# AliaksandrSiarohin/wc-gan

Hardware: AMD Instinct MI355X
Metric: images/sec G+D step, CIFAR-10 ResNet-SN+WC, batch 64 (higher is better)
Workload: dtype f32; 1 GPU; CIFAR-10 ResNet SN uncond + WC (scripts/cifar10_resnet_sn_uncond.sh), batch 64/GPU, training_ratio 5, generator_batch_multiple 2; parallelism=dp1, wc_statistics=per-replica, launch=hipgraph

## Files before the change

### include/wc_hip.h

```cpp
#ifndef WC_HIP_H
#define WC_HIP_H

#include <stddef.h>
#include <stdint.h>

#ifdef __cplusplus
extern "C" {
#endif

#define WC_ABI_VERSION 8

#define WC_OK                 0
#define WC_ERR_NULL          -1
#define WC_ERR_SHAPE         -2
#define WC_ERR_CHANNELS      -3
#define WC_ERR_WORKSPACE     -4
#define WC_ERR_ARG           -5

typedef void* wc_stream_t;

int         wc_abi_version(void);
const char* wc_error_string(int code);

#define WC_CORE_API "wc_stats_f32 wc_factor_f64 wc_color_f32 wc_group_bias_f32 wc_apply_f32 wc_apply_act_f32 " \
// ... 234 lines not shown

#define WC_CONV_SCRATCH_BYTES 2048

int wc_conv_supported(const wc_conv_geom* g);

int wc_conv_split_f32(const float* x, int64_t n, int relu, void* hi, void* lo, float* scale, void* amax_scratch,
                      wc_stream_t stream);

#define WC_CONV_COLSUM_ROWS 512
int wc_conv_split_colsum_f32(const float* x, int64_t n, int relu, void* hi, void* lo, float* scale, void* amax_scratch,
                             float* colsum_partials, int C, wc_stream_t stream);

#define WC_CONV_HIST_FLOATS (4 * 512 + 16)
#define WC_CONV_HIST_REDO (4 * 512)
int wc_conv_split_hist_f32(const float* x, int64_t n, int relu, void* hi, void* lo, float* scale, float* colsum_partials , int C,
                           float* hist, int bootstrap, wc_stream_t stream);

size_t wc_conv_weights_bytes(const wc_conv_geom* g);
int wc_conv_weights_f32(const float* w, int64_t stride_k, int64_t stride_n, int64_t stride_r, int64_t stride_s,
                        int64_t n_elems, const wc_conv_geom* g, void* image, float* scale, void* amax_scratch,
                        const float* known_amax, int known_count, wc_stream_t stream);

int wc_conv_weights_pair_f32(const float* w, int64_t stride_r, int64_t stride_s, int64_t n_elems,
                             int64_t a_stride_k, int64_t a_stride_n, const wc_conv_geom* ga, void* image_a,
                             int64_t b_stride_k, int64_t b_stride_n, const wc_conv_geom* gb, void* image_b,
                             float* scale, void* amax_scratch, const float* known_amax, int known_count,
                             wc_stream_t stream);

size_t wc_conv_workspace_bytes(const wc_conv_geom* g);
int wc_conv_f16x3(const void* xhi, const void* xlo, const float* xscale, const void* wimage, const float* wscale,
                  const float* bias, const void* zero_line, const wc_conv_geom* g, int relu, float* y,
                  void* ws, size_t ws_bytes, wc_stream_t stream);

size_t wc_conv_wrw_workspace_bytes(const wc_conv_geom* g);
int wc_conv_wrw_f16x3(const void* xhi, const void* xlo, const float* xscale, const void* ghi, const void* glo,
                      const float* gscale, const void* zero_line, const wc_conv_geom* g, float* dw, int64_t stride_k,
                      int64_t stride_n, int64_t stride_r, int64_t stride_s, void* ws, size_t ws_bytes,
                      wc_stream_t stream);

int    wc_conv_wrw_narrow_supported(int64_t N, int64_t H, int64_t W, int Cin, int Cout, int ksize);
size_t wc_conv_wrw_narrow_workspace_bytes(int64_t N, int64_t H, int64_t W, int Cin, int Cout, int ksize);
int    wc_conv_wrw_narrow_f32(const float* x, const float* gy, int64_t N, int64_t H, int64_t W, int Cin, int Cout, int ksize,
                              float* dw, int64_t stride_k, int64_t stride_n, int64_t stride_r, int64_t stride_s, float* db ,
                              void* ws, size_t ws_bytes, wc_stream_t stream);

int    wc_conv_fwd_narrow_f32(const float* x, const float* w, int64_t stride_k, int64_t stride_n, int64_t stride_r, int64_t stride_s,
                              const float* bias , int64_t N, int64_t H, int64_t W, int Cin, int Cout, int ksize, int relu,
                              float* y, wc_stream_t stream);

int wc_conv_wrw_bias_f16x3(const void* xhi, const void* xlo, const float* xscale, const void* ghi, const void* glo,
                           const float* gscale, const void* zero_line, const wc_conv_geom* g, float* dw, int64_t stride_k,
                           int64_t stride_n, int64_t stride_r, int64_t stride_s, const float* colsum_partials, float* db,
                           void* ws, size_t ws_bytes, wc_stream_t stream);

int wc_stream_copy_f32(const float* src, float* dst, int64_t n, wc_stream_t stream);

#ifdef __cplusplus
}
#endif
#endif
```

### wc_gan_amd/_lib.py

```python
from __future__ import annotations

import ctypes
import os
from ctypes import c_float, c_char_p, c_double, c_int, c_int64, c_size_t, c_void_p

_HERE = os.path.dirname(os.path.abspath(__file__))
LIB_PATH = os.path.join(_HERE, "libwc_hip.so")

WC_OK = 0
ABI_VERSION = 8
ERRORS = {-1: "WC_ERR_NULL", -2: "WC_ERR_SHAPE", -3: "WC_ERR_CHANNELS", -4: "WC_ERR_WORKSPACE", -5: "WC_ERR_ARG"}

SIGNATURES = {
    "wc_abi_version": (c_int, []),
    "wc_error_string": (c_char_p, [c_int]),
    "wc_stats_workspace_bytes": (c_size_t, [c_int64, c_int, c_int]),
    "wc_factor_workspace_bytes": (c_size_t, [c_int, c_int]),
    "wc_color_workspace_bytes": (c_size_t, [c_int, c_int]),
    "wc_bwd_reduce_workspace_bytes": (c_size_t, [c_int64, c_int64, c_int, c_int, c_int]),
    "wc_bwd_factor_workspace_bytes": (c_size_t, [c_int, c_int]),
    "wc_apply_workspace_bytes": (c_size_t, [c_int64, c_int64, c_int, c_int]),
    "wc_apply_plan_bytes": (c_size_t, [c_int, c_int]),
    "wc_bwd_apply_workspace_bytes": (c_size_t, [c_int64, c_int64, c_int, c_int]),
    "wc_stats_f32": (c_int, [c_void_p, c_int64, c_int, c_int, c_void_p, c_void_p, c_void_p, c_size_t, c_void_p]),
# ... 90 lines not shown
    "wc_stream_copy_f32": (c_int, [c_void_p, c_void_p, c_int64, c_void_p]),
    "wc_spectral_norm_workspace_bytes": (c_size_t, [c_int, c_int]),
    "wc_spectral_norm_batched_f32": (c_int, [c_void_p, c_int, c_int, c_float, c_void_p]),
    "wc_spectral_norm_bwd_batched_f32": (c_int, [c_void_p, c_int, c_int, c_void_p]),
    "wc_spectral_norm_f32": (c_int, [c_void_p, c_int, c_int, c_void_p, c_void_p, c_int, c_float, c_void_p, c_void_p,
                                     c_void_p, c_void_p, c_void_p, c_size_t, c_void_p]),
    "wc_spectral_norm_bwd_f32": (c_int, [c_void_p, c_void_p, c_void_p, c_void_p, c_void_p, c_int, c_int, c_int, c_void_p,
                                         c_void_p, c_size_t, c_void_p]),
    "wc_conv_supported": (c_int, [c_void_p]),
    "wc_conv_split_f32": (c_int, [c_void_p, c_int64, c_int, c_void_p, c_void_p, c_void_p, c_void_p, c_void_p]),
    "wc_conv_weights_bytes": (c_size_t, [c_void_p]),
    "wc_conv_weights_f32": (c_int, [c_void_p, c_int64, c_int64, c_int64, c_int64, c_int64, c_void_p, c_void_p, c_void_p,
                                    c_void_p, c_void_p, c_int, c_void_p]),
    "wc_spectral_norm_amax_offset": (c_size_t, [c_int, c_int]),
    "wc_spectral_norm_error_offset": (c_size_t, [c_int, c_int]),
    "wc_conv_split_hist_f32": (c_int, [c_void_p, c_int64, c_int, c_void_p, c_void_p, c_void_p, c_void_p, c_int, c_void_p, c_int, c_void_p]),
    "wc_conv_fwd_narrow_f32": (c_int, [c_void_p, c_void_p, c_int64, c_int64, c_int64, c_int64, c_void_p, c_int64, c_int64, c_int64, c_int, c_int, c_int,
                                       c_int, c_void_p, c_void_p]),
    "wc_conv_wrw_narrow_supported": (c_int, [c_int64, c_int64, c_int64, c_int, c_int, c_int]),
    "wc_conv_wrw_narrow_workspace_bytes": (c_size_t, [c_int64, c_int64, c_int64, c_int, c_int, c_int]),
    "wc_conv_wrw_narrow_f32": (c_int, [c_void_p, c_void_p, c_int64, c_int64, c_int64, c_int, c_int, c_int, c_void_p, c_int64, c_int64, c_int64,
                                       c_int64, c_void_p, c_void_p, c_size_t, c_void_p]),
    "wc_conv_split_colsum_f32": (c_int, [c_void_p, c_int64, c_int, c_void_p, c_void_p, c_void_p, c_void_p, c_void_p, c_int, c_void_p]),
    "wc_conv_wrw_bias_f16x3": (c_int, [c_void_p, c_void_p, c_void_p, c_void_p, c_void_p, c_void_p, c_void_p, c_void_p, c_void_p,
                                       c_int64, c_int64, c_int64, c_int64, c_void_p, c_void_p, c_void_p, c_size_t, c_void_p]),
    "wc_conv_weights_pair_f32": (c_int, [c_void_p, c_int64, c_int64, c_int64, c_int64, c_int64, c_void_p, c_void_p,
                                         c_int64, c_int64, c_void_p, c_void_p, c_void_p, c_void_p, c_void_p, c_int, c_void_p]),
    "wc_conv_wrw_workspace_bytes": (c_size_t, [c_void_p]),
    "wc_conv_wrw_f16x3": (c_int, [c_void_p, c_void_p, c_void_p, c_void_p, c_void_p, c_void_p, c_void_p, c_void_p, c_void_p,
                                  c_int64, c_int64, c_int64, c_int64, c_void_p, c_size_t, c_void_p]),
    "wc_conv_workspace_bytes": (c_size_t, [c_void_p]),
    "wc_conv_f16x3": (c_int, [c_void_p, c_void_p, c_void_p, c_void_p, c_void_p, c_void_p, c_void_p, c_void_p, c_int,
                              c_void_p, c_void_p, c_size_t, c_void_p]),
}



class SnItem(ctypes.Structure):
    _fields_ = [("W", c_void_p), ("u", c_void_p), ("v", c_void_p), ("w_sn", c_void_p), ("sigma", c_void_p),
                ("u_used", c_void_p), ("v_used", c_void_p), ("ws", c_void_p), ("rows", c_int), ("cols", c_int)]


class SnBwdItem(ctypes.Structure):
    _fields_ = [("g", c_void_p), ("w_sn", c_void_p), ("u", c_void_p), ("v", c_void_p), ("sigma", c_void_p),
                ("dW", c_void_p), ("ws", c_void_p), ("rows", c_int), ("cols", c_int)]


class ConvGeom(ctypes.Structure):
    _fields_ = [("N", c_int), ("H", c_int), ("W", c_int), ("Hin", c_int), ("Win", c_int), ("Cin", c_int),
                ("Hout", c_int), ("Wout", c_int), ("Cout", c_int), ("in_stride", c_int), ("out_stride", c_int),
                ("ntaps", c_int), ("nphase", c_int),
                ("dy", (ctypes.c_byte * 16) * 4), ("dx", (ctypes.c_byte * 16) * 4),
                ("off_y", ctypes.c_byte * 4), ("off_x", ctypes.c_byte * 4),
                ("nsrc", (ctypes.c_byte * 16) * 4),
                ("wr", ((ctypes.c_byte * 4) * 16) * 4), ("ws", ((ctypes.c_byte * 4) * 16) * 4),
                ("wcoef", c_float)]


_lib = None


class WcHipError(RuntimeError):
    pass


def shared_gpu_guard(device_count=None) -> bool:
# ... 53 lines not shown
```

### wc_gan_amd/conv.py

```python
from __future__ import annotations

import ctypes
import os

import torch
import torch.nn.functional as F

from . import _lib, _state
from .ops import _ptr, _stream

_zero_lines = {}


def _zero_line(device):
    z = _zero_lines.get(device)
    if z is None:
        z = _zero_lines[device] = torch.zeros(64, dtype=torch.uint8, device=device)
    return z


def _plain(r, s):
    return [(r, s)], 1.0


# ... 32 lines not shown


def _phase_geom(N, Hin, Win, Cin, Cout, source=_plain):
    g = _lib.ConvGeom()
    g.N, g.Hin, g.Win, g.Cin, g.Cout = N, Hin, Win, Cin, Cout
    g.H, g.W, g.Hout, g.Wout = Hin, Win, 2 * Hin, 2 * Win
    g.in_stride, g.out_stride, g.ntaps, g.nphase = 1, 2, 4, 4
    for py in range(2):
        for px in range(2):
            p = py * 2 + px
            g.off_y[p], g.off_x[p] = py, px
            t = 0
            for dy in ((-1, 0) if py == 0 else (0, 1)):
                for dx in ((-1, 0) if px == 0 else (0, 1)):
                    g.dy[p][t], g.dx[p][t] = dy, dx
                    _set_sources(g, p, t, py + 1 - 2 * dy, px + 1 - 2 * dx, source)
                    t += 1
    return g


def _supported(g):
    return bool(_lib.load().wc_conv_supported(ctypes.addressof(g)))


def supported(x, w, kind):
    handed = getattr(x, '_wc_planes', None) is not None
    if not (x.is_cuda and x.dtype == torch.float32 and x.dim() == 4 and (handed or x.is_contiguous()) and w.dtype == torch.float32):
        return False
    p = _plan(kind, x, w)
    return bool(p) and p.ok


class _Plan:
    __slots__ = ('ok', 'fwd', 'bwd', 'fwd_ws', 'bwd_ws', 'wrw_ws', 'fwd_ptr', 'bwd_ptr')

    def __init__(self, kind, N, H, W, wshape):
        class _W:
            shape = wshape
        lib = _lib.load()
        (gf, kf, nf), (gb, kb, nb) = _geoms(kind, N, H, W, _W)
        self.fwd, self.bwd = (gf, kf, nf), (gb, kb, nb)
        self.fwd_ptr, self.bwd_ptr = ctypes.addressof(gf), ctypes.addressof(gb)
        self.ok = bool(lib.wc_conv_supported(self.fwd_ptr)) and bool(lib.wc_conv_supported(self.bwd_ptr))
        self.fwd_ws = lib.wc_conv_workspace_bytes(self.fwd_ptr) if self.ok else 0
        self.bwd_ws = lib.wc_conv_workspace_bytes(self.bwd_ptr) if self.ok else 0
        self.wrw_ws = lib.wc_conv_wrw_workspace_bytes(self.fwd_ptr) if self.ok else 0


_plans = {}


def _plan(kind, x, w):
    key = (kind, tuple(x.shape), tuple(w.shape))
    p = _plans.get(key)
    if p is None:
        N, H, W, C = x.shape
        good = (kind == 'same' and w.shape[1] == C and w.shape[2] == w.shape[3] and w.shape[2] in (1, 3)) or \
               (kind == 'down' and w.shape[1] == C and tuple(w.shape[2:]) == (4, 4) and H % 2 == 0 and W % 2 == 0) or \
               (kind == 'down3' and w.shape[1] == C and tuple(w.shape[2:]) == (3, 3) and H % 2 == 0 and W % 2 == 0) or \
               (kind == 'up3' and w.shape[1] == C and tuple(w.shape[2:]) == (3, 3)) or \
               (kind == 'up' and w.shape[0] == C and tuple(w.shape[2:]) == (4, 4))
        if kind not in ('same', 'down', 'up', 'down3', 'up3'):
            raise ValueError(kind)
        p = _plans[key] = _Plan(kind, N, H, W, tuple(w.shape)) if good else False
    return p


def _colsum_ok(C):
    return C % 4 == 0 and 256 % (C // 4) == 0


SPLIT_HIST = os.environ.get('WC_SPLIT_HIST', '1') != '0'
HIST_FLOATS = 4 * 512 + 16
HIST_REDO = 4 * 512


_REDO_MODE = os.environ.get('WC_SPLIT_HIST_REDO', '1')


# ... 51 lines not shown
    ext = _storage_extent(w)
    if ext != w.numel():
        raise ValueError("weight must be dense")
    known = getattr(w, '_wc_amax', None)
    _lib.check(lib.wc_conv_weights_f32(_ptr(w), w.stride(k_axis), w.stride(n_axis), w.stride(2), w.stride(3), ext,
                                       ctypes.addressof(geom), _ptr(img), _ptr(scale), scale.data_ptr() + 4,
                                       _ptr(known), 0 if known is None else known.numel(), _stream()),
               "wc_conv_weights_f32")
    return img, scale


def weight_image_pair(w, fwd, bwd):
    lib = _lib.load()
    (ga, ka, na), (gb, kb, nb) = fwd, bwd
    img_a = torch.empty(lib.wc_conv_weights_bytes(ctypes.addressof(ga)), dtype=torch.uint8, device=w.device)
    img_b = torch.empty(lib.wc_conv_weights_bytes(ctypes.addressof(gb)), dtype=torch.uint8, device=w.device)
    scale = torch.empty(2 + 512, dtype=torch.float32, device=w.device)
    ext = _storage_extent(w)
    if ext != w.numel():
        raise ValueError("weight must be dense")
    known = getattr(w, '_wc_amax', None)
    _lib.check(lib.wc_conv_weights_pair_f32(_ptr(w), w.stride(2), w.stride(3), ext,
                                            w.stride(ka), w.stride(na), ctypes.addressof(ga), _ptr(img_a),
                                            w.stride(kb), w.stride(nb), ctypes.addressof(gb), _ptr(img_b),
                                            _ptr(scale), scale.data_ptr() + 8, _ptr(known), 0 if known is None else known.numel(),
                                            _stream()), "wc_conv_weights_pair_f32")
    return (img_a, scale[0:1]), (img_b, scale[1:2])


def _cached_image(w, key, geom, k_axis, n_axis):
    return weight_image(w, geom, k_axis, n_axis)


def run(planes, image, geom, bias=None, relu=False, nbytes=None):
    hi, lo, xs = planes
    img, ws = image
    lib = _lib.load()
    y = torch.empty((geom.N, geom.Hout, geom.Wout, geom.Cout), dtype=torch.float32, device=hi.device)
    if nbytes is None:
        nbytes = lib.wc_conv_workspace_bytes(ctypes.addressof(geom))
    work = torch.empty(nbytes, dtype=torch.uint8, device=hi.device) if nbytes else None
    _lib.check(lib.wc_conv_f16x3(_ptr(hi), _ptr(lo), _ptr(xs), _ptr(img), _ptr(ws), _ptr(bias) if bias is not None else None,
                                 _ptr(_zero_line(hi.device)), ctypes.addressof(geom), 1 if relu else 0, _ptr(y),
                                 _ptr(work), nbytes, _stream()), "wc_conv_f16x3")
    return y


def _geoms(kind, N, H, W, w):
    if kind == 'same':
        co, ci, k = w.shape[0], w.shape[1], w.shape[2]
        fwd = _dense_geom(N, H, W, ci, co, k, 1)
        bwd = _dense_geom(N, H, W, co, ci, k, 1)
        for t in range(k * k):
            bwd.dy[0][t], bwd.dx[0][t] = -bwd.dy[0][t], -bwd.dx[0][t]
        return (fwd, 1, 0), (bwd, 0, 1)
    if kind in ('down', 'down3'):
        co, ci = w.shape[0], w.shape[1]
        src = _pooled3 if kind == 'down3' else _plain
        return (_dense_geom(N, H, W, ci, co, 4, 2, src), 1, 0), (_phase_geom(N, H // 2, W // 2, co, ci, src), 0, 1)
    if kind == 'up3':
        co, ci = w.shape[0], w.shape[1]
        return (_phase_geom(N, H, W, ci, co, _upsampled3), 1, 0), (_dense_geom(N, 2 * H, 2 * W, co, ci, 4, 2, _upsampled3), 0, 1)
    ci, co = w.shape[0], w.shape[1]
    return (_phase_geom(N, H, W, ci, co), 0, 1), (_dense_geom(N, 2 * H, 2 * W, co, ci, 4, 2), 1, 0)


def weight_gradient(x_planes, g_planes, geom, w, k_axis, n_axis, nbytes=None, colsum=None):
    lib = _lib.load()
    xh, xl, xs = x_planes
    gh, gl, gs = g_planes[:3]
    dw = torch.empty_like(w)
    if dw.stride() != w.stride():
        raise ValueError("weight must be dense")
    if nbytes is None:
        nbytes = lib.wc_conv_wrw_workspace_bytes(ctypes.addressof(geom))
    ws = torch.empty(nbytes, dtype=torch.uint8, device=w.device)
    if colsum is not None:
        db = torch.empty(geom.Cout, dtype=torch.float32, device=w.device)
        _lib.check(lib.wc_conv_wrw_bias_f16x3(_ptr(xh), _ptr(xl), _ptr(xs), _ptr(gh), _ptr(gl), _ptr(gs), _ptr(_zero_line(w.device)),
                                              ctypes.addressof(geom), _ptr(dw), w.stride(k_axis), w.stride(n_axis), w.stride(2),
                                              w.stride(3), _ptr(colsum), _ptr(db), _ptr(ws), nbytes, _stream()),
                   "wc_conv_wrw_bias_f16x3")
        return dw, db
    _lib.check(lib.wc_conv_wrw_f16x3(_ptr(xh), _ptr(xl), _ptr(xs), _ptr(gh), _ptr(gl), _ptr(gs), _ptr(_zero_line(w.device)),
                                     ctypes.addressof(geom), _ptr(dw), w.stride(k_axis), w.stride(n_axis), w.stride(2),
                                     w.stride(3), _ptr(ws), nbytes, _stream()), "wc_conv_wrw_f16x3")
    return dw


def takes_planes(shape, wshape, kind):
    class _S:
        pass
    xs, ws = _S(), _S()
    xs.shape, ws.shape = tuple(shape), tuple(wshape)
    p = _plan(kind, xs, ws)
    return bool(p) and p.ok


class _FastConv(torch.autograd.Function):
    @staticmethod
    def forward(ctx, x, w, bias, kind, plan, relu_input=False, handed=None, site=None):
        gf, kf, nf = plan.fwd
        planes = handed if handed is not None else split_planes(x, relu=relu_input, site=site, role='x')
        ctx.site = site
        if ctx.needs_input_grad[0]:
            img, ctx.bwd_image = weight_image_pair(w, plan.fwd, plan.bwd)
        else:
            img, ctx.bwd_image = weight_image(w, gf, kf, nf), None
        y = run(planes, img, gf, bias, nbytes=plan.fwd_ws)
        ctx.save_for_backward(w, *planes, *((x,) if relu_input else ()))
        ctx.kind, ctx.has_bias, ctx.plan, ctx.relu_input = kind, bias is not None, plan, relu_input
        return y

    @staticmethod
    def backward(ctx, gy):
        w, xh, xl, xs = ctx.saved_tensors[:4]
        kind, plan = ctx.kind, ctx.plan
        gy = gy.contiguous()
        want_db = ctx.has_bias and ctx.needs_input_grad[2]
        fused_db = want_db and ctx.needs_input_grad[1] and _colsum_ok(gy.shape[-1])
        g_planes = split_planes(gy, colsum=fused_db, site=ctx.site, role='g')
        dx = dw = db = None
        if ctx.needs_input_grad[0]:
            gb, kb, nb = plan.bwd
            image = ctx.bwd_image if ctx.bwd_image is not None else weight_image(w, gb, kb, nb)
            dx = run(g_planes[:3], image, gb, nbytes=plan.bwd_ws)
            if ctx.relu_input:
                dx = torch.ops.aten.threshold_backward(dx, ctx.saved_tensors[4], 0)
        if ctx.needs_input_grad[1]:
            gf, kf, nf = plan.fwd
            if fused_db:
                dw, db = weight_gradient((xh, xl, xs), g_planes, gf, w, kf, nf, nbytes=plan.wrw_ws, colsum=g_planes[3])
            else:
                dw = weight_gradient((xh, xl, xs), g_planes, gf, w, kf, nf, nbytes=plan.wrw_ws)
        if want_db and not fused_db:
            db = gy.sum((0, 1, 2))
        return dx, dw, db, None, None, None, None, None


_ones = {}


def _one(device):
    t = _ones.get(device)
    if t is None:
        t = torch.ones(1, dtype=torch.float32, device=device)
        if not torch.cuda.is_current_stream_capturing():
            _ones[device] = t
    return t


class _SplitConv(torch.autograd.Function):

    @staticmethod
    def forward(ctx, x, w, bias, plan, st, site=None):
        from . import ops
        ctx.site = site
        gf, kf, nf = plan.fwd
        wf, bf = ops.fold_channel_scale(w, bias, st.scale, st.center)
        img = weight_image(wf, gf, kf, nf)
        ctx.bwd_image = None
        if ctx.needs_input_grad[0]:
            gb, kb, nb = plan.bwd
            ctx.bwd_image = weight_image(w, gb, kb, nb)
        hi, lo = st.planes[0].view(st.shape), st.planes[1].view(st.shape)
        one = _one(hi.device)
        y = run((hi, lo, one), img, gf, bf, nbytes=plan.fwd_ws)
        ctx.save_for_backward(w, hi, lo, one, st.scale, st.center)
        ctx.plan, ctx.has_bias = plan, bias is not None
        return y

    @staticmethod
    def backward(ctx, gy):
        from . import ops
        w, xh, xl, one, scale, center = ctx.saved_tensors
        plan = ctx.plan
        gy = gy.contiguous()
        need_w = ctx.needs_input_grad[1]
        need_b = ctx.has_bias and ctx.needs_input_grad[2]
        fused_db = need_w and _colsum_ok(gy.shape[-1])
        g_planes = split_planes(gy, colsum=fused_db, site=ctx.site, role='g')
        dx = dw = db = None
        if ctx.needs_input_grad[0]:
            gb, kb, nb = plan.bwd
            image = ctx.bwd_image if ctx.bwd_image is not None else weight_image(w, gb, kb, nb)
            dx = run(g_planes[:3], image, gb, nbytes=plan.bwd_ws)
        if need_w:
            gf, kf, nf = plan.fwd
            if fused_db:
                D, db = weight_gradient((xh, xl, one), g_planes, gf, w, kf, nf, nbytes=plan.wrw_ws, colsum=g_planes[3])
            else:
                D = weight_gradient((xh, xl, one), g_planes, gf, w, kf, nf, nbytes=plan.wrw_ws)
                db = gy.sum((0, 1, 2))
            dw = ops.unfold_channel_scale(D, db, scale, center)
        elif need_b:
            db = gy.sum((0, 1, 2))
        return dx, dw, (db if need_b else None), None, None, None


def split_conv(x, st, w, bias=None, site=None):
    p = _plan('same', x, w)
    if not (p and p.ok and tuple(w.shape[2:]) == (1, 1) and w.dtype == torch.float32):
        raise _lib.WcHipError(f"split_conv: a pre-split handle reached a convolution without a planes path {tuple(x.shape)} x {tuple(w.shape)}")
    return _SplitConv.apply(x, w, bias, p, st, site)


def fast_conv_or_none(x, w, bias=None, kind='same', relu_input=False, site=None):
    handed = getattr(x, '_wc_planes', None)
    if not supported(x, w, kind):
        if handed is not None:
            raise _lib.WcHipError(f"fast_conv: a K3 handle reached a convolution that cannot take planes {tuple(x.shape)} x {tuple(w.shape)} ({kind})")
        return None
    if handed is not None:
        if relu_input:
            raise ValueError("a K3 handle is already ReLU'd")
        return _FastConv.apply(x, w, bias, kind, _plan(kind, x, w), False, handed, site)
    return _FastConv.apply(x, w, bias, kind, _plan(kind, x, w), relu_input, None, site)


# ... 100 lines not shown
```

### wc_gan_amd/csrc/wc_conv.hip

```cpp
#include "wc_common.h"
#include "../../include/wc_hip.h"
#include <stdlib.h>


namespace {

constexpr int kMaxTaps = 16, kMaxPhase = 4;

struct ConvArgs {
    const _Float16* xhi; const _Float16* xlo;
    const _Float16* zero;
    const char* wimg;
    const float* xscale; const float* wscale;
    const float* bias;
    float* y;
    int N, H, W, Hin, Win, Cin, Cout, in_stride, ntaps, nphase, Hout, Wout, out_stride, relu;
    unsigned magHW, shHW, magW, shW;
    int ksplit; float* partial;
    signed char dy[kMaxPhase][kMaxTaps], dx[kMaxPhase][kMaxTaps];
    signed char offy[kMaxPhase], offx[kMaxPhase];
};

__device__ __forceinline__ void lds_dma16(const void* g, unsigned lds)
{
    unsigned keep;
    asm volatile("s_mov_b32 %0, m0\n\ts_mov_b32 m0, %2\n\ts_nop 0\n\tglobal_load_lds_dwordx4 %1, off\n\ts_mov_b32 m0, %0"
                 : "=&s"(keep) : "v"(g), "s"(lds) : "memory");
}

template <int MB, int NB, bool KS>
__global__ __launch_bounds__(256) void conv_f16x3_kernel(ConvArgs a)
{
    extern __shared__ __attribute__((aligned(16))) char smem[];
    constexpr int TM = 64 * MB, TN = 64 * NB;
    constexpr int A_BYTES = 2 * MB * 4 * 1024, B_BYTES = 2 * NB * 4 * 1024, STAGE = A_BYTES + B_BYTES;
    constexpr int AQ = (2 * MB) / 4;
    static_assert(AQ >= 1, "MB >= 2");

    const int tid = threadIdx.x, lane = tid & 63;
    const int wave = __builtin_amdgcn_readfirstlane(tid >> 6);
    const int wm = wave >> 1, wn = wave & 1;
    const int ntn = a.Cout / TN;
    const int phase = blockIdx.y / ntn, nt = blockIdx.y - phase * ntn;
    const unsigned m0 = blockIdx.x * TM;
    const unsigned HW = a.H * a.W;
    const int koff = (lane >> 5) * 8;

    int gy[AQ], gx[AQ];
    unsigned gpix[AQ];
    #pragma unroll
    for (int q = 0; q < AQ; ++q) {
        const unsigned m = m0 + (wave * AQ + q) * 32 + (lane & 31);
        const unsigned n = __umulhi(m, a.magHW) >> a.shHW, rem = m - n * HW;
        const unsigned yy = __umulhi(rem, a.magW) >> a.shW, xx = rem - yy * a.W;
        gy[q] = yy * a.in_stride; gx[q] = xx * a.in_stride; gpix[q] = n * (a.Hin * a.Win);
    }
    const unsigned lds0 = (unsigned)(size_t)((__attribute__((address_space(3))) char*)smem);
    const int nchunk = a.Cin >> 5;
    const int iters = a.ntaps * nchunk;
    const int nblk_all = a.Cout >> 5;
// ... 98 lines not shown
            #pragma unroll
            for (int g = 0; g < PER; ++g) {
                const int prod = g / (MB * NB), i = (g / NB) % MB, j = g % NB;
                acc[i][j] = __builtin_amdgcn_mfma_f32_32x32x16_f16(fa[ks][i][prod == 0 ? 1 : 0], fb[ks][j][prod == 1 ? 1 : 0], acc[i][j], 0, 0, 0);
                if ((g + 1) % GAP == 0) {
                    dma(ks * HALF + g / GAP);
                    __builtin_amdgcn_sched_barrier(0);
                }
                if (ks == 0 && g == PER / 2) {
                    frags(stage, 1);
                    __builtin_amdgcn_sched_barrier(0);
                }
            }
        }
    }
    __builtin_amdgcn_s_waitcnt(0x0F70);
    const float inv = 1.0f / (a.xscale[0] * a.wscale[0]);
    const int oy0 = a.offy[phase], ox0 = a.offx[phase];
    float bj[NB];
    #pragma unroll
    for (int j = 0; j < NB; ++j) bj[j] = a.bias ? a.bias[nt * TN + (wn * NB + j) * 32 + (lane & 31)] : 0.f;
    #pragma unroll
    for (int i = 0; i < MB; ++i) {
        #pragma unroll
        for (int r = 0; r < 16; ++r) {
            const unsigned row = (r & 3) + 8 * (r >> 2) + 4 * (lane >> 5);
            const unsigned m = m0 + (wm * MB + i) * 32 + row;
            const unsigned n = __umulhi(m, a.magHW) >> a.shHW, rem = m - n * HW;
            const unsigned yy = __umulhi(rem, a.magW) >> a.shW, xx = rem - yy * a.W;
            const int64_t opix = ((int64_t)n * a.Hout + (yy * a.out_stride + oy0)) * a.Wout + (xx * a.out_stride + ox0);
            const int64_t oe = opix * a.Cout + nt * TN + wn * NB * 32 + (lane & 31);
            if (KS) {
                float* o = a.partial + (int64_t)blockIdx.z * ((int64_t)a.N * a.Hout * a.Wout * a.Cout) + oe;
                #pragma unroll
                for (int j = 0; j < NB; ++j) o[j * 32] = acc[i][j][r];
            } else {
                float* o = a.y + oe;
                #pragma unroll
                for (int j = 0; j < NB; ++j) {
                    float v = acc[i][j][r] * inv + bj[j];
                    if (a.relu) v = fmaxf(v, 0.f);
                    o[j * 32] = v;
                }
            }
        }
    }
}

__global__ __launch_bounds__(256) void conv_ksplit_reduce_kernel(const float* __restrict__ partial, int ksplit, int64_t n4, int cout,
                                                                 const float* __restrict__ xscale, const float* __restrict__ wscale,
                                                                 const float* __restrict__ bias, int relu, float* __restrict__ y)
{
    const float inv = 1.0f / (xscale[0] * wscale[0]);
    for (int64_t i = (int64_t)blockIdx.x * 256 + threadIdx.x; i < n4; i += (int64_t)gridDim.x * 256) {
        f32x4 v = *reinterpret_cast<const f32x4*>(partial + 4 * i);
        int z = 1;
        for (; z + 3 < ksplit; z += 4) {
            f32x4 t[4];
            #pragma unroll
            for (int u = 0; u < 4; ++u) t[u] = *reinterpret_cast<const f32x4*>(partial + 4 * ((z + u) * n4 + i));
            #pragma unroll
            for (int u = 0; u < 4; ++u) v += t[u];
        }
        for (; z < ksplit; ++z) v += *reinterpret_cast<const f32x4*>(partial + 4 * (z * n4 + i));
        v = v * inv;
        if (bias) v += *reinterpret_cast<const f32x4*>(bias + (4 * i) % cout);
        if (relu) { v[0] = fmaxf(v[0], 0.f); v[1] = fmaxf(v[1], 0.f); v[2] = fmaxf(v[2], 0.f); v[3] = fmaxf(v[3], 0.f); }
        *reinterpret_cast<f32x4*>(y + 4 * i) = v;
    }
}

constexpr int kAmaxBlocks = 512;

__global__ __launch_bounds__(256) void conv_absmax_kernel(const float* __restrict__ x, int64_t n4, int64_t n, float* __restrict__ partial,
                                                          float* __restrict__ colsum = nullptr, int c4n = 0)
{
    __shared__ float red[4];
    __shared__ f32x4 red4[256];
    float m = 0.f;
    f32x4 cs = {0.f, 0.f, 0.f, 0.f};
    for (int64_t i = blockIdx.x * 256 + threadIdx.x; i < n4; i += (int64_t)gridDim.x * 256) {
        const f32x4 v = *reinterpret_cast<const f32x4*>(x + 4 * i);
        m = fmaxf(fmaxf(m, fabsf(v[0])), fmaxf(fabsf(v[1]), fmaxf(fabsf(v[2]), fabsf(v[3]))));
        cs += v;
    }
    if (blockIdx.x == 0 && threadIdx.x == 0) for (int64_t i = 4 * n4; i < n; ++i) m = fmaxf(m, fabsf(x[i]));
    #pragma unroll
    for (int o = 32; o > 0; o >>= 1) m = fmaxf(m, __shfl_xor(m, o));
    if ((threadIdx.x & 63) == 0) red[threadIdx.x >> 6] = m;
    if (colsum) red4[threadIdx.x] = cs;
    __syncthreads();
    if (threadIdx.x == 0) partial[blockIdx.x] = fmaxf(fmaxf(red[0], red[1]), fmaxf(red[2], red[3]));
    if (colsum && (int)threadIdx.x < c4n) {
        f32x4 t = red4[threadIdx.x];
        for (int p = threadIdx.x + c4n; p < 256; p += c4n) t += red4[p];
        *reinterpret_cast<f32x4*>(colsum + (int64_t)blockIdx.x * 4 * c4n + 4 * threadIdx.x) = t;
    }
}

__device__ __forceinline__ float scale_of(const float* __restrict__ partial, float mul = 1.0f, int count = kAmaxBlocks)
{
// ... 829 lines not shown
    if (!g) return 0;
    if (g->ntaps < 1 || g->ntaps > kMaxTaps || g->nphase < 1 || g->nphase > kMaxPhase) return 0;
    if ((g->Cin & 31) || (g->Cout & 127)) return 0;
    const int64_t M = (int64_t)g->N * g->H * g->W;
    if (M <= 0 || (M & 127) || M > (int64_t)1 << 31) return 0;
    if ((int64_t)g->N * g->Hin * g->Win > (int64_t)1 << 31) return 0;
    if (g->W < 2 || g->H < 1) return 0;
    return 1;
}

constexpr int kKsplitMaxWgs = 96;
constexpr int kKsplitTargetWgs = 256;
constexpr int kWrwTargetWgs = 512;

static int conv_ksplit(const wc_conv_geom* g)
{
    const int64_t M = (int64_t)g->N * g->H * g->W;
    const bool wide = (g->Cout % 256) == 0;
    const int64_t wgs = (M / 128) * g->nphase * (g->Cout / (wide ? 256 : 128));
    const int iters = g->ntaps * (g->Cin / 32);
    if (wgs > kKsplitMaxWgs || iters < 8) return 1;
    int k = (int)((kKsplitTargetWgs + wgs - 1) / wgs);
    if (k > iters / 4) k = iters / 4;
    return k < 1 ? 1 : (k > 8 ? 8 : k);
}

size_t wc_conv_workspace_bytes(const wc_conv_geom* g)
{
    if (!g) return 0;
    const int k = conv_ksplit(g);
    return k > 1 ? (size_t)k * g->N * g->Hout * g->Wout * g->Cout * 4 : 0;
}

int wc_conv_f16x3(const void* xhi, const void* xlo, const float* xscale, const void* wimage, const float* wscale,
                  const float* bias, const void* zero_line, const wc_conv_geom* g, int relu, float* y,
                  void* ws, size_t ws_bytes, wc_stream_t stream)
{
    hipStream_t st = (hipStream_t)stream;
    if (!xhi || !xlo || !xscale || !wimage || !wscale || !zero_line || !g || !y) return WC_ERR_ARG;
    if (!wc_conv_supported(g)) return WC_ERR_SHAPE;
    ConvArgs a;
    a.xhi = (const _Float16*)xhi; a.xlo = (const _Float16*)xlo; a.zero = (const _Float16*)zero_line;
    a.wimg = (const char*)wimage; a.xscale = xscale; a.wscale = wscale; a.bias = bias; a.y = y;
    a.N = g->N; a.H = g->H; a.W = g->W; a.Hin = g->Hin; a.Win = g->Win; a.Cin = g->Cin; a.Cout = g->Cout;
    a.in_stride = g->in_stride; a.ntaps = g->ntaps; a.nphase = g->nphase; a.Hout = g->Hout; a.Wout = g->Wout;
    a.out_stride = g->out_stride; a.relu = relu;
    a.ksplit = conv_ksplit(g); a.partial = (float*)ws;
    magic_u31((unsigned)(g->H * g->W), &a.magHW, &a.shHW);
    magic_u31((unsigned)g->W, &a.magW, &a.shW);
    if (a.ksplit > 1 && (!ws || ws_bytes < wc_conv_workspace_bytes(g))) return WC_ERR_WORKSPACE;
    for (int p = 0; p < kMaxPhase; ++p) {
        a.offy[p] = g->off_y[p]; a.offx[p] = g->off_x[p];
        for (int t = 0; t < kMaxTaps; ++t) { a.dy[p][t] = g->dy[p][t]; a.dx[p][t] = g->dx[p][t]; }
    }
    const int64_t M = (int64_t)g->N * g->H * g->W;
    const bool wide = (g->Cout % 256) == 0;
    const int64_t wgs_big = (M / 256) * g->nphase * (g->Cout / (wide ? 256 : 128));
    hipError_t e;
    if (a.ksplit == 1 && (M % 256) == 0 && wgs_big >= 256) e = wide ? launch_conv<4, 4>(a, st) : launch_conv<4, 2>(a, st);
    else if (a.ksplit > 1)                                  e = wide ? launch_conv<2, 4, true>(a, st) : launch_conv<2, 2, true>(a, st);
    else                                                    e = wide ? launch_conv<2, 4>(a, st) : launch_conv<2, 2>(a, st);
    if (e != hipSuccess) return (int)e;
    if (a.ksplit > 1) {
        const int64_t n4 = (int64_t)g->N * g->Hout * g->Wout * g->Cout / 4;
        hipLaunchKernelGGL(conv_ksplit_reduce_kernel, dim3(grid_for(n4)), dim3(256), 0, st, (const float*)ws, a.ksplit, n4, g->Cout,
                           xscale, wscale, bias, relu, y);
    }
    return (int)hipGetLastError();
}

static int wrw_splits(const wc_conv_geom* g, int* tile)
{
    const bool wide = (g->Cin % 256 == 0) && (g->Cout % 256 == 0) && g->nphase * g->ntaps * (g->Cin / 256) * (g->Cout / 256) >= 4;
    *tile = wide ? 256 : 128;
    const int tiles = g->nphase * g->ntaps * (g->Cin / *tile) * (g->Cout / *tile);
    const int64_t nchunks = (int64_t)g->N * g->H * g->W / 32;
    int splits = kWrwTargetWgs / tiles / 8 * 8;
    if (splits < 8) splits = 8;
    if (splits > 64) splits = 64;
    if (splits > nchunks) splits = (int)nchunks;
    return splits < 1 ? 1 : splits;
}

int wc_conv_wrw_narrow_supported(int64_t N, int64_t H, int64_t W, int Cin, int Cout, int ksize);

int wc_conv_fwd_narrow_f32(const float* x, const float* w, int64_t stride_k, int64_t stride_n, int64_t stride_r, int64_t stride_s,
                           const float* bias, int64_t N, int64_t H, int64_t W, int Cin, int Cout, int ksize, int relu, float* y, wc_stream_t stream)
{
    if (!x || !w || !y) return WC_ERR_ARG;
    if (!wc_conv_wrw_narrow_supported(N, H, W, Cin, Cout, ksize) || N * H * W * Cin >= ((int64_t)1 << 31)) return WC_ERR_SHAPE;
    hipStream_t st = (hipStream_t)stream;
    NarrowFwdArgs a = {};
    a.x = x; a.w = w; a.bias = bias; a.y = y;
    a.N = (int)N; a.H = (int)H; a.W = (int)W; a.Cin = Cin; a.Cout = Cout; a.ks = ksize; a.nrow = ksize * ksize * Cin; a.relu = relu;
    a.sk = stride_k; a.sn = stride_n; a.sr = stride_r; a.ss = stride_s;
    magic_u31((unsigned)(H * W), &a.magHW, &a.shHW);
    magic_u31((unsigned)W, &a.magW, &a.shW);
    for (int m = 0; m < 32; ++m) {
        const int tap = m < a.nrow ? m / Cin : 0, c = m < a.nrow ? m % Cin : 0;
        a.tr[m] = (signed char)(tap / ksize); a.ts[m] = (signed char)(tap % ksize); a.tch[m] = (signed char)c;
        a.tdy[m] = (signed char)(tap / ksize - ksize / 2); a.tdx[m] = (signed char)(tap % ksize - ksize / 2);
// ... 151 lines not shown
```

Measured before the change: 3586 images/sec.

## Fuse k-split conv reduction into last-arriving workgroup via atomic tile counters

For k-split forward/backward-data convolutions with narrow output channels, each workgroup stores its partial tile and bumps a per-tile atomic counter. The last workgroup to arrive sums the partials and applies scale, bias and relu itself, so the separate reduce kernel launch is skipped. Counter slots come from a per-stream slab that is pre-zeroed and reset by the finishing block, with per-capture slots under graph capture. This removes one launch and one full pass over the partial buffer per conv, at the cost of atomics, extra synchronisation and a serialized tail in the last block.

```diff
diff --git a/include/wc_hip.h b/include/wc_hip.h
--- a/include/wc_hip.h
+++ b/include/wc_hip.h
@@ -290,6 +290,11 @@
                   const float* bias, const void* zero_line, const wc_conv_geom* g, int relu, float* y,
                   void* ws, size_t ws_bytes, wc_stream_t stream);
 
+size_t wc_conv_counter_bytes(const wc_conv_geom* g);
+int wc_conv_f16x3_ex(const void* xhi, const void* xlo, const float* xscale, const void* wimage, const float* wscale,
+                     const float* bias, const void* zero_line, const wc_conv_geom* g, int relu, float* y,
+                     void* ws, size_t ws_bytes, unsigned* counters , size_t counter_bytes, wc_stream_t stream);
+
 size_t wc_conv_wrw_workspace_bytes(const wc_conv_geom* g);
 int wc_conv_wrw_f16x3(const void* xhi, const void* xlo, const float* xscale, const void* ghi, const void* glo,
                       const float* gscale, const void* zero_line, const wc_conv_geom* g, float* dw, int64_t stride_k,
diff --git a/wc_gan_amd/_lib.py b/wc_gan_amd/_lib.py
--- a/wc_gan_amd/_lib.py
+++ b/wc_gan_amd/_lib.py
@@ -146,6 +146,9 @@
     "wc_conv_workspace_bytes": (c_size_t, [c_void_p]),
     "wc_conv_f16x3": (c_int, [c_void_p, c_void_p, c_void_p, c_void_p, c_void_p, c_void_p, c_void_p, c_void_p, c_int,
                               c_void_p, c_void_p, c_size_t, c_void_p]),
+    "wc_conv_counter_bytes": (c_size_t, [c_void_p]),
+    "wc_conv_f16x3_ex": (c_int, [c_void_p, c_void_p, c_void_p, c_void_p, c_void_p, c_void_p, c_void_p, c_void_p, c_int,
+                                 c_void_p, c_void_p, c_size_t, c_void_p, c_size_t, c_void_p]),
 }
 
 
diff --git a/wc_gan_amd/conv.py b/wc_gan_amd/conv.py
--- a/wc_gan_amd/conv.py
+++ b/wc_gan_amd/conv.py
@@ -88,7 +88,7 @@
 
 
 class _Plan:
-    __slots__ = ('ok', 'fwd', 'bwd', 'fwd_ws', 'bwd_ws', 'wrw_ws', 'fwd_ptr', 'bwd_ptr')
+    __slots__ = ('ok', 'fwd', 'bwd', 'fwd_ws', 'bwd_ws', 'wrw_ws', 'fwd_ptr', 'bwd_ptr', 'fwd_cnt', 'bwd_cnt')
 
     def __init__(self, kind, N, H, W, wshape):
         class _W:
@@ -101,6 +101,8 @@
         self.fwd_ws = lib.wc_conv_workspace_bytes(self.fwd_ptr) if self.ok else 0
         self.bwd_ws = lib.wc_conv_workspace_bytes(self.bwd_ptr) if self.ok else 0
         self.wrw_ws = lib.wc_conv_wrw_workspace_bytes(self.fwd_ptr) if self.ok else 0
+        self.fwd_cnt = lib.wc_conv_counter_bytes(self.fwd_ptr) if self.ok else 0
+        self.bwd_cnt = lib.wc_conv_counter_bytes(self.bwd_ptr) if self.ok else 0
 
 
 _plans = {}
@@ -218,17 +220,63 @@
     return weight_image(w, geom, k_axis, n_axis)
 
 
-def run(planes, image, geom, bias=None, relu=False, nbytes=None):
+class _CounterSlab:
+    SLOT = 512
+    WORDS = 1 << 16
+
+    def __init__(self, device):
+        self.device = device
+        self.slab, self.used, self.by_stream, self.captured = None, 0, {}, []
+
+    def _take(self):
+        if self.slab is None or self.used + self.SLOT > 4 * self.WORDS:
+            if torch.cuda.is_current_stream_capturing():
+                return None
+            self.slab = torch.zeros(self.WORDS, dtype=torch.int32, device=self.device)
+            self.used = 0
+        p = self.slab.data_ptr() + self.used
+        self.used += self.SLOT
+        return (self.slab, p)
+
+    def slot(self, nbytes):
+        if nbytes > self.SLOT:
+            raise ValueError(f"k-split counters of {nbytes} bytes exceed a slot")
+        if torch.cuda.is_current_stream_capturing():
+            s = self._take()
+            if s is not None:
+                self.captured.append(s)
+        else:
+            st = _stream()
+            s = self.by_stream.get(st)
+            if s is None:
+                s = self.by_stream[st] = self._take()
+        return None if s is None else s[1]
+
+
+_counter_slabs = {}
+
+
+def _counters(device, nbytes):
+    c = _counter_slabs.get(device)
+    if c is None:
+        c = _counter_slabs[device] = _CounterSlab(device)
+    return c.slot(nbytes)
+
+
+def run(planes, image, geom, bias=None, relu=False, nbytes=None, counter_bytes=None):
     hi, lo, xs = planes
     img, ws = image
     lib = _lib.load()
     y = torch.empty((geom.N, geom.Hout, geom.Wout, geom.Cout), dtype=torch.float32, device=hi.device)
     if nbytes is None:
         nbytes = lib.wc_conv_workspace_bytes(ctypes.addressof(geom))
+    if counter_bytes is None:
+        counter_bytes = lib.wc_conv_counter_bytes(ctypes.addressof(geom))
     work = torch.empty(nbytes, dtype=torch.uint8, device=hi.device) if nbytes else None
-    _lib.check(lib.wc_conv_f16x3(_ptr(hi), _ptr(lo), _ptr(xs), _ptr(img), _ptr(ws), _ptr(bias) if bias is not None else None,
-                                 _ptr(_zero_line(hi.device)), ctypes.addressof(geom), 1 if relu else 0, _ptr(y),
-                                 _ptr(work), nbytes, _stream()), "wc_conv_f16x3")
+    cnt = _counters(hi.device, counter_bytes) if counter_bytes else None
+    _lib.check(lib.wc_conv_f16x3_ex(_ptr(hi), _ptr(lo), _ptr(xs), _ptr(img), _ptr(ws), _ptr(bias) if bias is not None else None,
+                                    _ptr(_zero_line(hi.device)), ctypes.addressof(geom), 1 if relu else 0, _ptr(y),
+                                    _ptr(work), nbytes, cnt, counter_bytes if cnt else 0, _stream()), "wc_conv_f16x3_ex")
     return y
 
 
@@ -293,7 +341,7 @@
             img, ctx.bwd_image = weight_image_pair(w, plan.fwd, plan.bwd)
         else:
             img, ctx.bwd_image = weight_image(w, gf, kf, nf), None
-        y = run(planes, img, gf, bias, nbytes=plan.fwd_ws)
+        y = run(planes, img, gf, bias, nbytes=plan.fwd_ws, counter_bytes=plan.fwd_cnt)
         ctx.save_for_backward(w, *planes, *((x,) if relu_input else ()))
         ctx.kind, ctx.has_bias, ctx.plan, ctx.relu_input = kind, bias is not None, plan, relu_input
         return y
@@ -310,7 +358,7 @@
         if ctx.needs_input_grad[0]:
             gb, kb, nb = plan.bwd
             image = ctx.bwd_image if ctx.bwd_image is not None else weight_image(w, gb, kb, nb)
-            dx = run(g_planes[:3], image, gb, nbytes=plan.bwd_ws)
+            dx = run(g_planes[:3], image, gb, nbytes=plan.bwd_ws, counter_bytes=plan.bwd_cnt)
             if ctx.relu_input:
                 dx = torch.ops.aten.threshold_backward(dx, ctx.saved_tensors[4], 0)
         if ctx.needs_input_grad[1]:
@@ -351,7 +399,7 @@
             ctx.bwd_image = weight_image(w, gb, kb, nb)
         hi, lo = st.planes[0].view(st.shape), st.planes[1].view(st.shape)
         one = _one(hi.device)
-        y = run((hi, lo, one), img, gf, bf, nbytes=plan.fwd_ws)
+        y = run((hi, lo, one), img, gf, bf, nbytes=plan.fwd_ws, counter_bytes=plan.fwd_cnt)
         ctx.save_for_backward(w, hi, lo, one, st.scale, st.center)
         ctx.plan, ctx.has_bias = plan, bias is not None
         return y
@@ -370,7 +418,7 @@
         if ctx.needs_input_grad[0]:
             gb, kb, nb = plan.bwd
             image = ctx.bwd_image if ctx.bwd_image is not None else weight_image(w, gb, kb, nb)
-            dx = run(g_planes[:3], image, gb, nbytes=plan.bwd_ws)
+            dx = run(g_planes[:3], image, gb, nbytes=plan.bwd_ws, counter_bytes=plan.bwd_cnt)
         if need_w:
             gf, kf, nf = plan.fwd
             if fused_db:
diff --git a/wc_gan_amd/csrc/wc_conv.hip b/wc_gan_amd/csrc/wc_conv.hip
--- a/wc_gan_amd/csrc/wc_conv.hip
+++ b/wc_gan_amd/csrc/wc_conv.hip
@@ -17,6 +17,7 @@
     int N, H, W, Hin, Win, Cin, Cout, in_stride, ntaps, nphase, Hout, Wout, out_stride, relu;
     unsigned magHW, shHW, magW, shW;
     int ksplit; float* partial;
+    unsigned* counters;
     signed char dy[kMaxPhase][kMaxTaps], dx[kMaxPhase][kMaxTaps];
     signed char offy[kMaxPhase], offx[kMaxPhase];
 };
@@ -26,6 +27,50 @@
     unsigned keep;
     asm volatile("s_mov_b32 %0, m0\n\ts_mov_b32 m0, %2\n\ts_nop 0\n\tglobal_load_lds_dwordx4 %1, off\n\ts_mov_b32 m0, %0"
                  : "=&s"(keep) : "v"(g), "s"(lds) : "memory");
+}
+
+__device__ __forceinline__ f32x4 ksplit_out(f32x4 v, float inv, const float* __restrict__ bias, int64_t ch, int relu)
+{
+    v = v * inv;
+    if (bias) v += *reinterpret_cast<const f32x4*>(bias + ch);
+    if (relu) { v[0] = fmaxf(v[0], 0.f); v[1] = fmaxf(v[1], 0.f); v[2] = fmaxf(v[2], 0.f); v[3] = fmaxf(v[3], 0.f); }
+    return v;
+}
+
+template <int K, int TM, int TN>
+__device__ __forceinline__ void ksplit_finish(const ConvArgs& a, int phase, int nt, unsigned m0, int tid)
+{
+    constexpr int C4 = TN / 4, RPP = 256 / C4, ROWS = TM / RPP;
+    constexpr int U = K <= 2 ? 8 : (K <= 4 ? 4 : 2);
+    static_assert(ROWS % U == 0, "whole row groups");
+    const int c4 = tid % C4, r0 = tid / C4;
+    const float inv = 1.0f / (a.xscale[0] * a.wscale[0]);
+    const int64_t plane = (int64_t)a.N * a.Hout * a.Wout * a.Cout;
+    const int64_t ch = (int64_t)nt * TN + 4 * c4;
+    const unsigned HW = a.H * a.W;
+    const int oy0 = a.offy[phase], ox0 = a.offx[phase];
+    for (int g = 0; g < ROWS; g += U) {
+        int64_t oe[U];
+        #pragma unroll
+        for (int u = 0; u < U; ++u) {
+            const unsigned m = m0 + r0 + RPP * (g + u);
+            const unsigned n = __umulhi(m, a.magHW) >> a.shHW, rem = m - n * HW;
+            const unsigned yy = __umulhi(rem, a.magW) >> a.shW, xx = rem - yy * a.W;
+            oe[u] = (((int64_t)n * a.Hout + (yy * a.out_stride + oy0)) * a.Wout + (xx * a.out_stride + ox0)) * a.Cout + ch;
+        }
+        f32x4 t[K][U];
+        #pragma unroll
+        for (int z = 0; z < K; ++z)
+            #pragma unroll
+            for (int u = 0; u < U; ++u) t[z][u] = *reinterpret_cast<const f32x4*>(a.partial + z * plane + oe[u]);
+        #pragma unroll
+        for (int u = 0; u < U; ++u) {
+            f32x4 v = t[0][u];
+            #pragma unroll
+            for (int z = 1; z < K; ++z) v += t[z][u];
+            *reinterpret_cast<f32x4*>(a.y + oe[u]) = ksplit_out(v, inv, a.bias, ch, a.relu);
+        }
+    }
 }
 
 template <int MB, int NB, bool KS>
@@ -190,8 +235,15 @@
             const int64_t oe = opix * a.Cout + nt * TN + wn * NB * 32 + (lane & 31);
             if (KS) {
                 float* o = a.partial + (int64_t)blockIdx.z * ((int64_t)a.N * a.Hout * a.Wout * a.Cout) + oe;
-                #pragma unroll
-                for (int j = 0; j < NB; ++j) o[j * 32] = acc[i][j][r];
+                if (a.counters) {
+                    #pragma unroll
+                    for (int j = 0; j < NB; ++j)
+                        __hip_atomic_store(reinterpret_cast<unsigned*>(o + j * 32), __float_as_uint(acc[i][j][r]), __ATOMIC_RELAXED,
+                                           __HIP_MEMORY_SCOPE_AGENT);
+                } else {
+                    #pragma unroll
+                    for (int j = 0; j < NB; ++j) o[j * 32] = acc[i][j][r];
+                }
             } else {
                 float* o = a.y + oe;
                 #pragma unroll
@@ -202,6 +254,32 @@
                 }
             }
         }
+    }
+    if (!KS || !a.counters) return;
+    asm volatile("s_waitcnt vmcnt(0)" ::: "memory");
+    __syncthreads();
+    int* last = reinterpret_cast<int*>(smem);
+    if (tid == 0) {
+        unsigned* cnt = a.counters + blockIdx.y * gridDim.x + blockIdx.x;
+        const unsigned ticket = __hip_atomic_fetch_add(cnt, 1u, __ATOMIC_RELAXED, __HIP_MEMORY_SCOPE_AGENT);
+        const int is_last = ticket == (unsigned)a.ksplit - 1;
+        if (is_last) {
+            __hip_atomic_store(cnt, 0u, __ATOMIC_RELAXED, __HIP_MEMORY_SCOPE_AGENT);
+            __builtin_amdgcn_fence(__ATOMIC_ACQUIRE, "agent");
+            asm volatile("s_waitcnt vmcnt(0)" ::: "memory");
+        }
+        *last = is_last;
+    }
+    __syncthreads();
+    if (!*last) return;
+    switch (a.ksplit) {
+        case 2: ksplit_finish<2, TM, TN>(a, phase, nt, m0, tid); break;
+        case 3: ksplit_finish<3, TM, TN>(a, phase, nt, m0, tid); break;
+        case 4: ksplit_finish<4, TM, TN>(a, phase, nt, m0, tid); break;
+        case 5: ksplit_finish<5, TM, TN>(a, phase, nt, m0, tid); break;
+        case 6: ksplit_finish<6, TM, TN>(a, phase, nt, m0, tid); break;
+        case 7: ksplit_finish<7, TM, TN>(a, phase, nt, m0, tid); break;
+        default: ksplit_finish<8, TM, TN>(a, phase, nt, m0, tid); break;
     }
 }
 
@@ -221,10 +299,7 @@
             for (int u = 0; u < 4; ++u) v += t[u];
         }
         for (; z < ksplit; ++z) v += *reinterpret_cast<const f32x4*>(partial + 4 * (z * n4 + i));
-        v = v * inv;
-        if (bias) v += *reinterpret_cast<const f32x4*>(bias + (4 * i) % cout);
-        if (relu) { v[0] = fmaxf(v[0], 0.f); v[1] = fmaxf(v[1], 0.f); v[2] = fmaxf(v[2], 0.f); v[3] = fmaxf(v[3], 0.f); }
-        *reinterpret_cast<f32x4*>(y + 4 * i) = v;
+        *reinterpret_cast<f32x4*>(y + 4 * i) = ksplit_out(v, inv, bias, (4 * i) % cout, relu);
     }
 }
 
@@ -1120,20 +1195,29 @@
     return k > 1 ? (size_t)k * g->N * g->Hout * g->Wout * g->Cout * 4 : 0;
 }
 
-int wc_conv_f16x3(const void* xhi, const void* xlo, const float* xscale, const void* wimage, const float* wscale,
-                  const float* bias, const void* zero_line, const wc_conv_geom* g, int relu, float* y,
-                  void* ws, size_t ws_bytes, wc_stream_t stream)
+size_t wc_conv_counter_bytes(const wc_conv_geom* g)
+{
+    if (!g || !wc_conv_supported(g) || conv_ksplit(g) == 1 || (g->Cout % 256) == 0) return 0;
+    const int64_t M = (int64_t)g->N * g->H * g->W;
+    const int64_t tiles = (M / 128) * g->nphase * (g->Cout / 128);
+    return (size_t)((tiles * 4 + 15) & ~(int64_t)15);
+}
+
+int wc_conv_f16x3_ex(const void* xhi, const void* xlo, const float* xscale, const void* wimage, const float* wscale,
+                     const float* bias, const void* zero_line, const wc_conv_geom* g, int relu, float* y,
+                     void* ws, size_t ws_bytes, unsigned* counters, size_t counter_bytes, wc_stream_t stream)
 {
     hipStream_t st = (hipStream_t)stream;
     if (!xhi || !xlo || !xscale || !wimage || !wscale || !zero_line || !g || !y) return WC_ERR_ARG;
     if (!wc_conv_supported(g)) return WC_ERR_SHAPE;
+    if (counters && counter_bytes < wc_conv_counter_bytes(g)) return WC_ERR_WORKSPACE;
     ConvArgs a;
     a.xhi = (const _Float16*)xhi; a.xlo = (const _Float16*)xlo; a.zero = (const _Float16*)zero_line;
     a.wimg = (const char*)wimage; a.xscale = xscale; a.wscale = wscale; a.bias = bias; a.y = y;
     a.N = g->N; a.H = g->H; a.W = g->W; a.Hin = g->Hin; a.Win = g->Win; a.Cin = g->Cin; a.Cout = g->Cout;
     a.in_stride = g->in_stride; a.ntaps = g->ntaps; a.nphase = g->nphase; a.Hout = g->Hout; a.Wout = g->Wout;
     a.out_stride = g->out_stride; a.relu = relu;
-    a.ksplit = conv_ksplit(g); a.partial = (float*)ws;
+    a.ksplit = conv_ksplit(g); a.partial = (float*)ws; a.counters = wc_conv_counter_bytes(g) ? counters : nullptr;
     magic_u31((unsigned)(g->H * g->W), &a.magHW, &a.shHW);
     magic_u31((unsigned)g->W, &a.magW, &a.shW);
     if (a.ksplit > 1 && (!ws || ws_bytes < wc_conv_workspace_bytes(g))) return WC_ERR_WORKSPACE;
@@ -1149,12 +1233,19 @@
     else if (a.ksplit > 1)                                  e = wide ? launch_conv<2, 4, true>(a, st) : launch_conv<2, 2, true>(a, st);
     else                                                    e = wide ? launch_conv<2, 4>(a, st) : launch_conv<2, 2>(a, st);
     if (e != hipSuccess) return (int)e;
-    if (a.ksplit > 1) {
+    if (a.ksplit > 1 && !a.counters) {
         const int64_t n4 = (int64_t)g->N * g->Hout * g->Wout * g->Cout / 4;
         hipLaunchKernelGGL(conv_ksplit_reduce_kernel, dim3(grid_for(n4)), dim3(256), 0, st, (const float*)ws, a.ksplit, n4, g->Cout,
                            xscale, wscale, bias, relu, y);
     }
     return (int)hipGetLastError();
+}
+
+int wc_conv_f16x3(const void* xhi, const void* xlo, const float* xscale, const void* wimage, const float* wscale,
+                  const float* bias, const void* zero_line, const wc_conv_geom* g, int relu, float* y,
+                  void* ws, size_t ws_bytes, wc_stream_t stream)
+{
+    return wc_conv_f16x3_ex(xhi, xlo, xscale, wimage, wscale, bias, zero_line, g, relu, y, ws, ws_bytes, nullptr, 0, stream);
 }
 
 static int wrw_splits(const wc_conv_geom* g, int* tile)
```

Measured after the change: 3558 images/sec (median of 2 runs). Within noise of the previous version (-0.8%).
